# KumarRobotics/top_down_renderer

Hardware: AMD Instinct MI355X
Metric: particle-updates/sec (render+score+resample) (higher is better)
Workload: dtype f32

## Files before the change

include/tdr.h:

```cpp
#ifndef TDR_H_
#define TDR_H_

#include <stddef.h>
#include <stdint.h>

#ifdef __cplusplus
extern "C" {
#endif

#define TDR_OK 0
#define TDR_ERR_ARG (-1)
#define TDR_ERR_HIP (-2)
#define TDR_ERR_NOMEM (-3)

#define TDR_MAX_CLASSES 15
#define TDR_ST_FIELDS 7
enum { TDR_ST_INIT_X = 0, TDR_ST_INIT_Y = 1, TDR_ST_DX = 2, TDR_ST_DY = 3, TDR_ST_THETA = 4, TDR_ST_SCALE = 5,
       TDR_ST_HAVE_INIT = 6 };

typedef struct tdr_state {
  float init_x_px, init_y_px, dx_m, dy_m, theta, scale;
  uint8_t have_init;
  uint8_t pad_[3];
} tdr_state;
// ... 173 lines not shown
int tdr_k_local_map_polar(const tdr_map_desc* map, const float* tab, int nb, int nr, float cx, float cy, float scale,
                          float res, float* dists_out, uint8_t* mask_out, void* stream);
int tdr_k_local_map_cart(const tdr_map_desc* map, int rows, int cols, float cx, float cy, float rot, float res,
                         float* dists_out, uint8_t* mask_out, void* stream);

int tdr_k_active_diffs(const tdr_map_desc* map, const float* tab, int nb, int nr, float res, const float* centres,
                       const int32_t* shifts, int K, int ncand, double* sums_out, void* stream);
int tdr_active_candidates_host(const float* preds, int K, int nb, float* centres, float* dists, float* thetas,
                               int32_t* shifts, int* ntheta_out, int* ndist_out);

#define TDR_MEAN_COV_FLOATS 4800
int tdr_k_mean_cov(const float* st, int64_t cap, int64_t n, const float* about, float* out, void* stream);
int tdr_k_set_scale(float* st, int64_t cap, int64_t n, const float* scale_dev, void* stream);
int tdr_k_save_ml_state(const float* info, const float* st, int64_t cap, int64_t src_shard, int64_t n, float* out12,
                        void* stream);
int tdr_k_shift_init(float* st, int64_t cap, int64_t n, float dx, float dy, void* stream);

int tdr_config_compact(int on);
int tdr_config_shift_uniform(int mode);
float tdr_config_shift_uniform_span(float cells);
int tdr_config_ray_split(int k);
int tdr_config_cart_skip(int on);
int tdr_config_init_mfma(int on);
int tdr_config_uw_waves(int on);
int64_t tdr_shift_uniform_launches(void);

int tdr_profile_enable(int on);
int tdr_profile_score_ms(double* total_ms, int64_t* launches);
int tdr_profile_shares(double* dense_ms, double* scattered_ms, int64_t* scattered_particles);
int tdr_profile_variants(int64_t out[16]);

int64_t tdr_config_tuning(const char* name, int64_t value);
int tdr_su_tail_plan(int nchunks, int k, int q, int row, int* group, int* s0, int* s1);
int tdr_selftest_score(void);
int tdr_k_selftest_round(const float* x, int64_t n, float limit, int32_t* out, void* stream);
int tdr_libm_variant(void);
int tdr_libm_force_variant(int variant);
int tdr_sincosf_host(const float* x, int64_t n, int variant, float* sin_out, float* cos_out);
int tdr_k_selftest_sincos(const float* x, int64_t n, float* sin_out, float* cos_out, void* stream);
int tdr_logf_host(const float* x, int64_t n, float* out);
int tdr_k_selftest_logf(const float* x, int64_t n, float* out, void* stream);
int tdr_k_selftest_atan2(const float* y, const float* x, int64_t n, float* out, void* stream);

int tdr_k_states_aos_to_soa(const tdr_state* aos, int64_t n, float* st, int64_t cap, void* stream);
int tdr_k_states_soa_to_aos(const float* st, int64_t cap, int64_t n, tdr_state* aos, void* stream);
size_t tdr_locality_tmp_ints(int64_t n, int map_rows, int map_cols);
int tdr_k_locality_order(const float* st, int64_t cap, int64_t n, int map_rows, int map_cols, int32_t* perm_out,
                         int32_t* keys_tmp, void* stream);
size_t tdr_locality_pose_tmp_ints(int64_t n);
int tdr_k_locality_order_pose(const float* st, int64_t cap, int64_t n, int map_rows, int map_cols, float theta_radius,
                              int32_t* perm_out, int32_t* keys_tmp, void* stream);

typedef struct tdr_map tdr_map;
typedef struct tdr_renderer tdr_renderer;
typedef struct tdr_filter tdr_filter;

int tdr_map_create(tdr_map** out);
void tdr_map_destroy(tdr_map* m);
int tdr_map_set(tdr_map* m, const float* class_maps, const uint8_t* class_mask, int ncls, int rows, int cols,
                float resolution, int center_x, int center_y);
int tdr_map_set_labels(tdr_map* m, const uint8_t* label_img, int img_h, int img_w, const int32_t* flatten_lut,
                       int lut_size, int ncls, float resolution, int center_x, int center_y);
int tdr_map_update_labels_incremental(tdr_map* m, const uint8_t* label_img, int img_h, int img_w,
                                      const int32_t* flatten_lut, int lut_size, int ncls, float resolution, int center_x,
                                      int center_y, int64_t* changed_cells);
int tdr_map_patch_labels(tdr_map* m, const uint8_t* patch, int y0, int x0, int h, int w, int center_x, int center_y,
// ... 144 lines not shown
```

top_down_renderer_amd/_lib.py:

```python
import ctypes as C
import os

_PKG = os.path.dirname(os.path.abspath(__file__))
SO_PATH = os.environ.get("TDR_LIB_PATH") or os.path.join(_PKG, "libtdr_hip.so")

TDR_ST_FIELDS = 7
TDR_MAX_CLASSES = 15
TDR_SVG_NO_KEY = 0xFFFFFFFF


class FilterParamsC(C.Structure):
    _fields_ = [
        ("pos_cov", C.c_float), ("theta_cov", C.c_float), ("regularization", C.c_float),
        ("init_pos_px_x", C.c_float), ("init_pos_px_y", C.c_float), ("init_pos_px_cov", C.c_float),
        ("init_pos_m_x", C.c_float), ("init_pos_m_y", C.c_float),
        ("init_pos_deg_theta", C.c_float), ("init_pos_deg_cov", C.c_float),
        ("force_on_map", C.c_int32),
        ("fixed_scale", C.c_float), ("scale_log_min", C.c_float), ("scale_log_max", C.c_float),
        ("num_classes", C.c_int32),
        ("class_weights", C.c_float * 16),
    ]


class MapDescC(C.Structure):
# ... 79 lines not shown
    "tdr_raster_workspace_bytes": (_i64, [_i64]),
    "tdr_k_raster_polar": (_i, [_vp, _i, _i, _i64, _f, _f, _vp, _i, _i, _i, _vp, _vp, _vp, _vp]),
    "tdr_k_raster_cart": (_i, [_vp, _i, _i, _i64, _f, _vp, _i, _i, _i, _vp, _vp, _vp, _vp]),
    "tdr_raster_geo_workspace_bytes": (_i64, [_i64]),
    "tdr_k_raster_geo_polar": (_i, [_vp, _i, _i64, _i64, _f, _f, _i, _i, _vp, _vp, _vp]),
    "tdr_k_raster_geo_cart": (_i, [_vp, _i, _i64, _i64, _f, _i, _i, _vp, _vp]),
    "tdr_k_pack_scan": (_i, [_vp, _i, _i, _i, _vp, _vp]),
    "tdr_score_workspace_floats": (C.c_size_t, [_i, _i, _i, _i64, _i64]),
    "tdr_k_score_polar": (_i, [C.POINTER(MapDescC), _vp, _vp, _i, _i, _f, C.POINTER(FilterParamsC), _vp, _i64, _i64,
                               _i64, _vp, _f, _i, _vp, _vp, _vp]),
    "tdr_k_active_diffs": (_i, [C.POINTER(MapDescC), _vp, _i, _i, _f, _vp, _vp, _i, _i, _vp, _vp]),
    "tdr_active_candidates_host": (_i, [_vp, _i, _i, _vp, _vp, _vp, _vp, C.POINTER(_i), C.POINTER(_i)]),
    "tdr_logf_host": (_i, [_vp, _i64, _vp]),
    "tdr_k_selftest_logf": (_i, [_vp, _i64, _vp, _vp]),
    "tdr_rng_pipe_create": (_i, [_i64, C.POINTER(_vp)]),
    "tdr_rng_pipe_destroy": (None, [_vp]),
    "tdr_rng_pipe_on_device": (_i, [_vp]),
    "tdr_rng_pipe_from_host": (_i, [_vp, _vp, _vp]),
    "tdr_rng_pipe_to_host": (_i, [_vp, _vp, _vp]),
    "tdr_rng_pipe_normals": (_i, [_vp, _i64, _i64, _i64, _i, C.POINTER(_vp), _vp]),
    "tdr_rng_pipe_uniform": (_i, [_vp, C.POINTER(_vp), _vp]),
    "tdr_rng_dev_workspace_bytes": (C.c_size_t, [_i64]),
    "tdr_k_rng_propagate_normals": (_i, [_vp, _i64, _i64, _i64, _i, _vp, _vp, _vp]),
    "tdr_k_rng_uniform": (_i, [_vp, _vp, _vp]),
    "tdr_rng_get_state_host": (_i, [_vp, _vp]),
    "tdr_rng_set_state_host": (_i, [_vp, _vp]),
    "tdr_k_resample_dev": (_i, [_vp, _i64, _i64, _vp, _i64, _i64, _vp, _vp]),
    "tdr_score_ctx_create": (_i, [C.POINTER(_vp)]),
    "tdr_score_ctx_destroy": (None, [_vp]),
    "tdr_score_ctx_span": (C.c_float, [_vp]),
    "tdr_score_ctx_trial_calls": (_i64, [_vp]),
    "tdr_config_tuning": (_i64, [C.c_char_p, _i64]),
    "tdr_su_tail_plan": (_i, [_i, _i, _i, _i, C.POINTER(_i), C.POINTER(_i), C.POINTER(_i)]),
    "tdr_selftest_score": (_i, []),
    "tdr_profile_variants": (_i, [C.POINTER(_i64)]),
    "tdr_score_ctx_set_polar_factors": (_i, [_vp, _vp, _i, _i]),
    "tdr_polar_factors_host": (_i, [_i, _i, _f, _f, _vp]),
    "tdr_k_score_polar_ctx": (_i, [C.POINTER(MapDescC), _vp, _vp, _i, _i, _f, C.POINTER(FilterParamsC), _vp, _i64, _i64,
                                   _i64, _vp, _f, _i, _vp, _vp, _vp, _vp]),
    "tdr_score_geo_workspace_floats": (C.c_size_t, [_i, _i, _i, _i64, _i64]),
    "tdr_k_score_polar_geo": (_i, [C.POINTER(MapDescC), C.POINTER(MapDescC), _vp, _vp, _vp, _f, _f, _i, _i, _f,
                                   C.POINTER(FilterParamsC), _vp, _i64, _i64, _i64, _vp, _f, _i, _vp, _vp, _vp]),
    "tdr_score_cart_workspace_floats": (C.c_size_t, [_i, _i, _i, _i64, _i64]),
    "tdr_k_score_cart": (_i, [C.POINTER(MapDescC), _vp, _i, _i, _f, C.POINTER(FilterParamsC), _vp, _i64, _i64, _i64,
                              _vp, _vp, _vp, _vp]),
    "tdr_score_cart_init_workspace_floats": (C.c_size_t, [_i, _i, _i, _i64, _i64]),
    "tdr_k_score_cart_init": (_i, [C.POINTER(MapDescC), _vp, _i, _i, _f, C.POINTER(FilterParamsC), _vp, _i64, _i64, _i64,
                                   _vp, _vp]),
    "tdr_k_propagate": (_i, [_vp, _i64, _i64, _vp, _f, _f, _f, _i, _f, _f, _vp, _u64, _u64, _i64, _vp]),
    "tdr_rng_create": (_vp, [_u32]),
    "tdr_rng_destroy": (None, [_vp]),
    "tdr_rng_uniform_host": (_f, [_vp]),
    "tdr_propagate_normals_host": (_i, [_vp, _i64, _i, _vp]),
    "tdr_k_update_weights": (_i, [_vp, _vp, _i64, _vp, _vp, _vp]),
    "tdr_prefix_workspace_bytes": (_i64, [_i64]),
    "tdr_k_prefix": (_i, [_vp, _i64, _vp, _vp, _vp]),
    "tdr_k_prefix_mode": (_i, [_vp, _i64, _i, _vp, _vp, _vp, _vp]),
    "tdr_k_resample": (_i, [_vp, _i64, _i64, _f, _i64, _i64, _vp, _vp]),
    "tdr_k_gather_states": (_i, [_vp, _i64, _i64, _vp, _i64, _vp, _i64, _vp]),
    "tdr_init_particles_host": (_i, [_vp, _vp, _i, _i, _i, _f, C.POINTER(FilterParamsC), _i, _vp, C.POINTER(C.c_int64)]),
    "tdr_init_particles_count": (_i64, [C.POINTER(FilterParamsC), _i]),
    "tdr_init_workspace_bytes": (C.c_size_t, []),
    "tdr_k_init_particles": (_i, [_vp, C.POINTER(MapDescC), C.POINTER(FilterParamsC), _i, _i64, _i64, _vp, _i64,
                                  C.POINTER(C.c_int64), _vp, _vp]),
    "tdr_rng_pipe_init_particles": (_i, [_vp, C.POINTER(MapDescC), C.POINTER(FilterParamsC), _i, _i64, _i64, _vp, _i64,
                                         C.POINTER(C.c_int64), _vp, _vp]),
# ... 123 lines not shown
```

top_down_renderer_amd/csrc/tdr_score.hip:

```cpp

#include "tdr_common.h"
#include "tdr_batch.h"
#include "tdr_sincosf.h"

struct ScoreArgs {
  const float* rec;
  int rows, cols;
  float resolution;
  const float* tab;
  const float* utab = nullptr;
  const float* scan_pk;
  int nb, nr;
  float res;
  const float* st;
  int64_t cap, n;
  const int32_t* order;
  const int32_t* count = nullptr;
  const int32_t* slot_base = nullptr;
  int use_theta_override = 0;
  float theta_override = 0.f;
  int only_uninit = 0;
  int group, nchunks;
  int64_t npad;
  float* part;
// ... 591 lines not shown
      }
    cost = cost / (float)norm;
  }
  a.raw_w[p] = (float)(1. / (double)(cost + a.fp.regularization));
}

static int finalize_tlog(int nchunks, int64_t nslots) {
  int tl = 0;
  while (tl < 4 && (nchunks >> (tl + 1)) >= 4 && (nslots << (tl + 1)) <= 131072) tl++;
  return tl;
}
static void launch_finalize(FinalizeArgs& f, int64_t nslots, hipStream_t s) {
  f.tlog = finalize_tlog(f.nchunks, nslots);
  hipLaunchKernelGGL(score_finalize_kernel, dim3((unsigned)cdiv(nslots << f.tlog, 256)), dim3(256), 0, s, f);
}

#define TDR_CART_WAVE_MUL 2
static int64_t g_score_waves = 131072;
static int g_score_group = 0;
static int g_su_group = 0;
static int64_t score_wave_target() { return g_score_waves; }
extern "C" int tdr_config_init_ahead(int);
extern "C" int tdr_config_batch_init_search(int);
extern "C" int tdr_config_prefix_head(int);
extern "C" int tdr_config_ray_block_major(int);
extern "C" int tdr_config_ray_patch(int);
extern "C" int tdr_config_ray_borrow(int);
extern "C" int tdr_config_cart_seg_rows(int);
extern "C" int tdr_config_mt_stretches(int);
extern "C" int tdr_config_su_wave_span(int);
extern "C" int tdr_config_su_lds_pad(int);
extern "C" int tdr_config_su_tail_groups(int);
extern "C" int tdr_config_su_tail_parts(int);
extern "C" int tdr_config_init_device(int);
extern "C" int64_t tdr_config_init_window_words(int64_t);
extern "C" int64_t tdr_config_cart_init_chunk(int64_t);
extern "C" int64_t tdr_config_tuning(const char* name, int64_t value) {
  if (!name) return -1;
  const std::string n(name);
  if (n == "score_waves") { if (value > 0) g_score_waves = value; return g_score_waves; }
  if (n == "score_group") { if (value >= 0) g_score_group = (int)value; return g_score_group; }
  if (n == "su_group") { if (value >= 0) g_su_group = (int)value; return g_su_group; }
  if (n == "batch_init_search") return tdr_config_batch_init_search((int)std::max<int64_t>(value, -1));
  if (n == "init_ahead") return tdr_config_init_ahead((int)std::min<int64_t>(std::max<int64_t>(value, -1), 3));
  if (n == "prefix_head") return tdr_config_prefix_head((int)std::max<int64_t>(value, -1));
  if (n == "ray_borrow") return tdr_config_ray_borrow((int)std::max<int64_t>(value, -1));
  if (n == "ray_patch") return tdr_config_ray_patch((int)std::max<int64_t>(value, -1));
  if (n == "ray_block_major") return tdr_config_ray_block_major((int)std::max<int64_t>(value, -1));
  if (n == "cart_seg_rows") return tdr_config_cart_seg_rows((int)std::max<int64_t>(value, -1));
  if (n == "mt_stretches") return tdr_config_mt_stretches((int)std::max<int64_t>(value, -1));
  if (n == "su_lds_pad") return tdr_config_su_lds_pad((int)std::max<int64_t>(value, -1));
  if (n == "su_tail_groups") return tdr_config_su_tail_groups((int)std::min<int64_t>(std::max<int64_t>(value, -1), 1 << 20));
  if (n == "su_tail_parts") return tdr_config_su_tail_parts((int)std::min<int64_t>(std::max<int64_t>(value, -1), 8));
  if (n == "su_wave_span") return tdr_config_su_wave_span((int)std::max<int64_t>(value, -1));
  if (n == "init_device") return tdr_config_init_device((int)std::max<int64_t>(value, -1));
  if (n == "init_window_words") return tdr_config_init_window_words(value > 0 ? value : -1);
  if (n == "cart_init_chunk") return tdr_config_cart_init_chunk(value > 0 ? value : -1);
  return -1;
}
static void choose_chunks(int64_t n, int nr, int& rpc, int& nchunks, int target_mul = 1) {
  int64_t nbatches = cdiv(std::max<int64_t>(n, 1), 64);
  int64_t want = std::max<int64_t>(1, cdiv(score_wave_target() * target_mul, nbatches));
  nchunks = (int)std::min<int64_t>(nr, want);
  rpc = (int)cdiv(nr, nchunks);
  nchunks = (int)cdiv(nr, rpc);
}

__global__ void utab_kernel(const float* __restrict__ tab, int64_t n2, float scale, float res,
                            float* __restrict__ utab) {
  const int64_t k = (int64_t)blockIdx.x * blockDim.x + threadIdx.x;
  if (k < n2) utab[k] = (tab[k] * scale) * res;
}

static int score_group_rings(int nb, int nr, int rf, int64_t n_total) {
  const int forced = g_score_group;
  const int64_t ring_bytes = std::max<int64_t>((int64_t)nb * rf * 4, 1);
  int g = (int)std::min<int64_t>(8, (32 * 1024) / ring_bytes);
  const int64_t chunks_wanted = cdiv(2048, cdiv(std::max<int64_t>(n_total, 1), 256));
  g = (int)std::min<int64_t>(g, std::max<int64_t>(1, nr / std::max<int64_t>(chunks_wanted, 1)));
  if (forced > 0) g = forced;
  g = std::max(1, std::min<int>(g, (int)((60 * 1024) / ring_bytes)));
  if (g >= TDR_SCORE_U) g -= g % TDR_SCORE_U;
  return std::max(g, 1);
}
extern "C" int tdr_cmap_words(int ncls);
struct ScoreWs {
// ... 679 lines not shown
```

top_down_renderer_amd/csrc/tdr_score_su.h:

```cpp
#ifndef TDR_SCORE_SU_H_
#define TDR_SCORE_SU_H_
#include "tdr_common.h"

static inline int64_t su_npad(int64_t n, int nb) { return cdiv(n + 63 * std::min<int64_t>(nb, n), 64) * 64; }
bool tdr_su_shape_ok(int nb, int nr, int group, int64_t n_total);
struct SuWs {
  int64_t tab_su, desc, bbox, keys_in, keys_out, vals_in, vals_out, ints, slots, sort_tmp, ray_tab, ray_desc, ray_multi, ray_rad, total;
  int64_t slots2, wave_tmp;
};
#define TDR_SU_TAIL_INTS 10
#define TDR_RAY_MAX_SPLIT 8
SuWs tdr_su_ws(int nb, int nr, int group, int64_t n);

#define TDR_SU_NSECT 8
__host__ __device__ static inline int su_tail_plan(int nchunks, int k, int q, int row, int* group, int* s0, int* s1) {
  const int lq = q >= 8 ? 3 : (q >= 4 ? 2 : (q >= 2 ? 1 : 0));
  const int kk = k < 0 ? 0 : (k > nchunks ? nchunks : k);
  const int head = nchunks - kk, rows = head + (kk << lq);
  if (row < 0 || row >= rows) return rows;
  if (row < head) {
    *group = row; *s0 = 0; *s1 = TDR_SU_NSECT;
  } else {
    const int t = row - head, part = t & ((1 << lq) - 1);
    *group = head + (t >> lq);
    *s0 = part << (3 - lq);
    *s1 = (part + 1) << (3 - lq);
  }
  return rows;
}
void tdr_su_tail(int nchunks, int64_t n, int* k, int* q);

struct SuLaunch {
  const tdr_map_desc* map;
  const float* tab;
  bool uniform_scale;
  const float* scan_pk;
  int nb, nr, rf;
  float res;
  const float* st;
  int64_t cap, n;
  const int32_t* perm;
// ... 37 lines not shown
```

top_down_renderer_amd/csrc/tdr_score_su.hip:

```cpp
#include <rocprim/device/device_radix_sort.hpp>

#include <atomic>

#include "tdr_score_dev.h"
#include "tdr_score_su.h"
#include "tdr_score_su_asm.h"

#define SU_CODE_FULL 0xFFu
#define SU_CODE_FULL_ALL 0xFEu
#define SU_CODE_PAD 0xFDu
#define SU_NSECT TDR_SU_NSECT
#define SU_BOX_WORDS 4096

struct SuArgs {
  const uint32_t* crec;
  const uint32_t* kmask;
  int kcolw;
  unsigned kmask_off;
  const uint32_t* dict_int;
  int dict_n, ctiles_r;
  int pkcol;
  const int32_t* inexact;
  int rows, cols;
  float resolution;
// ... 67 lines not shown
  desc[4 * t + 2] = ckc;
  desc[4 * t + 3] = sh | (((jj & 3) == 0 && anyfull) ? 0x80000000u : 0u);
}

__global__ __launch_bounds__(256) void su_bbox_kernel(const float* __restrict__ tab_su, int nb, int nr, int group,
                                                      float* __restrict__ bbox) {
  const int chunk = blockIdx.x, sect = blockIdx.y;
  const int i0 = (int)((int64_t)sect * nb / SU_NSECT), i1 = (int)((int64_t)(sect + 1) * nb / SU_NSECT);
  const int gn = min(nr - chunk * group, group);
  float lo0 = 3.402823466e+38f, hi0 = -3.402823466e+38f, lo1 = lo0, hi1 = hi0;
  const int cnt = (i1 - i0) * gn;
  for (int t = threadIdx.x; t < cnt; t += 256) {
    const int i = i0 + t / gn, jj = t % gn;
    const float* e = tab_su + (((int64_t)chunk * nb + i) * group + jj) * 2;
    lo0 = fminf(lo0, e[0]); hi0 = fmaxf(hi0, e[0]);
    lo1 = fminf(lo1, e[1]); hi1 = fmaxf(hi1, e[1]);
  }
  __shared__ float red[4][256];
  red[0][threadIdx.x] = lo0; red[1][threadIdx.x] = hi0; red[2][threadIdx.x] = lo1; red[3][threadIdx.x] = hi1;
  __syncthreads();
  for (int d = 128; d > 0; d >>= 1) {
    if ((int)threadIdx.x < d) {
      red[0][threadIdx.x] = fminf(red[0][threadIdx.x], red[0][threadIdx.x + d]);
      red[1][threadIdx.x] = fmaxf(red[1][threadIdx.x], red[1][threadIdx.x + d]);
      red[2][threadIdx.x] = fminf(red[2][threadIdx.x], red[2][threadIdx.x + d]);
      red[3][threadIdx.x] = fmaxf(red[3][threadIdx.x], red[3][threadIdx.x + d]);
    }
    __syncthreads();
  }
  if (threadIdx.x < 4) bbox[((int64_t)chunk * SU_NSECT + sect) * 4 + threadIdx.x] = red[threadIdx.x][0];
}

__global__ __launch_bounds__(256) void su_key_kernel(const float* __restrict__ st, int64_t cap, int64_t n,
                                                     const int32_t* __restrict__ perm, int nb, float span,
                                                     uint32_t* __restrict__ keys, int32_t* __restrict__ vals,
                                                     int* __restrict__ cnt) {
  extern __shared__ int hist[];
  for (int k = threadIdx.x; k <= nb; k += 256) hist[k] = 0;
  __syncthreads();
  const int64_t t = (int64_t)blockIdx.x * blockDim.x + threadIdx.x;
  if (t < n) {
    const int32_t p = perm ? perm[t] : (int32_t)t;
    uint32_t key = (uint32_t)rot_shift_dev(st[TDR_ST_THETA * cap + p], nb);
    if (span > 0.f) {
      auto centre = [&](int64_t q, float& x, float& y) {
        const float sc = st[TDR_ST_SCALE * cap + q];
        x = st[TDR_ST_DX * cap + q] * sc + st[TDR_ST_INIT_X * cap + q];
        y = st[TDR_ST_DY * cap + q] * sc + st[TDR_ST_INIT_Y * cap + q];
      };
      const int64_t ta = t >= 32 ? t - 32 : 0, tb = t + 32 < n ? t + 32 : n - 1;
      float x0, y0, x1, y1;
      centre(perm ? perm[ta] : ta, x0, y0);
      centre(perm ? perm[tb] : tb, x1, y1);
      if (!(fabsf(x1 - x0) <= span && fabsf(y1 - y0) <= span)) key = (uint32_t)nb;
    }
    keys[t] = key;
    vals[t] = p;
    atomicAdd(&hist[key], 1);
  }
  __syncthreads();
  for (int k = threadIdx.x; k <= nb; k += 256)
    if (hist[k]) atomicAdd(&cnt[k], hist[k]);
}

__global__ __launch_bounds__(256) void su_offsets_kernel(const int* __restrict__ cnt, int nkeys, int* __restrict__ start,
                                                         int* __restrict__ slot_start, int* __restrict__ counts) {
  __shared__ int sa[256], sb[256];
  int carry_a = 0, carry_b = 0;
  for (int base = 0; base < nkeys; base += 256) {
    const int k = base + threadIdx.x;
    const int c = k < nkeys ? cnt[k] : 0;
    const int cp = k < nkeys - 1 ? (c + 63) & ~63 : c;
    sa[threadIdx.x] = c;
    sb[threadIdx.x] = cp;
    __syncthreads();
    for (int d = 1; d < 256; d <<= 1) {
      const int va = threadIdx.x >= d ? sa[threadIdx.x - d] : 0;
      const int vb = threadIdx.x >= d ? sb[threadIdx.x - d] : 0;
      __syncthreads();
      sa[threadIdx.x] += va;
      sb[threadIdx.x] += vb;
      __syncthreads();
    }
    if (k < nkeys) {
      start[k] = carry_a + sa[threadIdx.x] - c;
      slot_start[k] = carry_b + sb[threadIdx.x] - cp;
    }
    carry_a += sa[255];
    carry_b += sb[255];
    __syncthreads();
  }
  if (threadIdx.x == 0) {
    const int sparse = cnt[nkeys - 1];
    counts[0] = carry_b - sparse;
    counts[1] = sparse;
    counts[2] = carry_b;
  }
}

__global__ __launch_bounds__(256) void su_scatter_kernel(const uint32_t* __restrict__ keys, const int32_t* __restrict__ vals,
                                                         int64_t n, const int* __restrict__ start,
                                                         const int* __restrict__ slot_start, int32_t* __restrict__ slots) {
  const int64_t t = (int64_t)blockIdx.x * blockDim.x + threadIdx.x;
  if (t >= n) return;
  const uint32_t k = keys[t];
  slots[slot_start[k] + ((int)t - start[k])] = vals[t];
}

__global__ __launch_bounds__(256) void su_wave_far_kernel(const float* __restrict__ st, int64_t cap, const int32_t* __restrict__ slots,
                                                          const int32_t* __restrict__ counts, float wave_span,
                                                          int32_t* __restrict__ keep, int32_t* __restrict__ moved) {
  const int lane = threadIdx.x & 63;
  const int64_t w = (int64_t)blockIdx.x * 4 + (threadIdx.x >> 6), base = w * 64;
  if (base >= (int64_t)counts[0]) return;
  const int32_t p = slots[base + lane];
  float x0 = 3.0e38f, x1 = -3.0e38f, y0 = 3.0e38f, y1 = -3.0e38f;
  if (p >= 0) {
    const float sc = st[TDR_ST_SCALE * cap + p];
    const float x = st[TDR_ST_DX * cap + p] * sc + st[TDR_ST_INIT_X * cap + p];
    const float y = st[TDR_ST_DY * cap + p] * sc + st[TDR_ST_INIT_Y * cap + p];
    x0 = x1 = x;
    y0 = y1 = y;
  }
#pragma unroll
  for (int d = 32; d > 0; d >>= 1) {
    x0 = fminf(x0, __shfl_xor(x0, d)); x1 = fmaxf(x1, __shfl_xor(x1, d));
    y0 = fminf(y0, __shfl_xor(y0, d)); y1 = fmaxf(y1, __shfl_xor(y1, d));
  }
  const int nvalid = __popcll(__ballot(p >= 0));
  const bool far = (x1 - x0 > wave_span) || (y1 - y0 > wave_span);
  if (lane == 0) {
    keep[w] = far ? 0 : 1;
    moved[w] = far ? nvalid : 0;
  }
}
__global__ __launch_bounds__(256) void su_compact_offsets_kernel(int32_t* __restrict__ keep, int32_t* __restrict__ moved,
                                                                 int32_t* __restrict__ counts, int32_t* __restrict__ old_counts) {
  __shared__ int sa[256], sb[256];
  const int c0 = counts[0], c1 = counts[1], c2 = counts[2];
// ... 606 lines not shown
extern "C" int64_t tdr_shift_uniform_launches(void) { return g_su_launches.load(); }
bool tdr_su_shape_ok(int nb, int nr, int group, int64_t n_total) {
  if (g_su_mode == 0) return false;
  if (group % 4 != 0 || nb > 4095) return false;
  if (g_su_mode == 2) return true;
  if ((int64_t)nb * nr < 8192) return false;
  return n_total >= (int64_t)64 * nb;
}
static int g_su_tail_groups = 4, g_su_tail_parts = 4;
extern "C" int tdr_config_su_tail_groups(int k) {
  if (k >= 0) g_su_tail_groups = k;
  return g_su_tail_groups;
}
extern "C" int tdr_config_su_tail_parts(int q) {
  if (q >= 0) g_su_tail_parts = q >= 8 ? 8 : (q >= 4 ? 4 : (q >= 2 ? 2 : 1));
  return g_su_tail_parts;
}
void tdr_su_tail(int nchunks, int64_t n, int* k, int* q) {
  *k = std::min(g_su_tail_groups, nchunks);
  *q = g_su_tail_parts;
  if (g_su_mode != 2 && cdiv(std::max<int64_t>(n, 1), 256) * nchunks < 2 * 256 * 6) *k = 0;
  if (*k == 0 || *q == 1) { *k = 0; *q = 1; }
}
extern "C" int tdr_su_tail_plan(int nchunks, int k, int q, int row, int* group, int* s0, int* s1) {
  int g = 0, a = 0, b = 0;
  const int rows = su_tail_plan(nchunks, k, q, row, &g, &a, &b);
  if (row >= 0 && row < rows) {
    if (group) *group = g;
    if (s0) *s0 = a;
    if (s1) *s1 = b;
  }
  return rows;
}
static size_t su_sort_tmp_bytes(int64_t n) {
  size_t bytes = 0;
  uint32_t* k = nullptr;
  int32_t* v = nullptr;
  hipError_t e = rocprim::radix_sort_pairs(nullptr, bytes, k, k, v, v, (size_t)std::max<int64_t>(n, 1), 0u, 12u,
                                           (hipStream_t)0, false);
  if (e != hipSuccess || bytes == 0) bytes = (size_t)(n + 4096) * 16;
  return bytes;
}
SuWs tdr_su_ws(int nb, int nr, int group, int64_t n) {
  SuWs w;
  const int64_t nchunks = cdiv(nr, group), nbins = nchunks * nb * group;
  int64_t o = 0;
  auto take = [&](int64_t words) { const int64_t at = o; o += (words + 63) / 64 * 64; return at; };
  w.tab_su = take(2 * nbins);
  w.desc = take(4 * nbins);
  w.bbox = take(nchunks * SU_NSECT * 4);
  w.keys_in = take(n);
  w.keys_out = take(n);
  w.vals_in = take(n);
  w.vals_out = take(n);
  w.ints = take(3 * ((int64_t)nb + 1) + TDR_SU_TAIL_INTS);
  w.slots = take(su_npad(n, nb));
  w.slots2 = take(su_npad(n, nb));
  w.wave_tmp = take(2 * (su_npad(n, nb) / 64 + 1));
  w.sort_tmp = take((int64_t)((su_sort_tmp_bytes(n) + 3) / 4));
  const int64_t T = tdr_ray_padded_samples(nb, nr);
  w.ray_tab = take(2 * T);
  w.ray_desc = take((T + 1) / 2);
  w.ray_multi = take((int64_t)nb * nr);
  w.ray_rad = take(T / nb);
  w.total = o;
  return w;
}

int tdr_su_order(const SuLaunch& L, const SuWs& W, hipStream_t s, const int32_t** slots_out, const int32_t** counts_out) {
  int32_t* base = L.ws;
  uint32_t* keys_in = reinterpret_cast<uint32_t*>(base + W.keys_in);
  uint32_t* keys_out = reinterpret_cast<uint32_t*>(base + W.keys_out);
  int32_t* vals_in = base + W.vals_in;
  int32_t* vals_out = base + W.vals_out;
  int* cnt = base + W.ints;
  const int nkeys = L.nb + 1;
  int* start = cnt + nkeys;
  int* slot_start = start + nkeys;
  int* counts = slot_start + nkeys;
  int32_t* slots = base + W.slots;
  const int64_t n = L.n;
  HIP_TRY(hipMemsetAsync(cnt, 0, sizeof(int) * (size_t)(3 * nkeys + TDR_SU_TAIL_INTS), s));
  HIP_TRY(hipMemsetAsync(slots, 0xFF, sizeof(int32_t) * (size_t)L.npad, s));
  hipLaunchKernelGGL(su_key_kernel, dim3((unsigned)cdiv(n, 256)), dim3(256), sizeof(int) * (size_t)nkeys, s, L.st, L.cap, n,
                     L.perm, L.nb, L.span, keys_in, vals_in, cnt);
  LAUNCH_CHECK("su_key");
  hipLaunchKernelGGL(su_offsets_kernel, dim3(1), dim3(256), 0, s, (const int*)cnt, nkeys, start, slot_start, counts);
  LAUNCH_CHECK("su_offsets");
  unsigned bits = 1;
  while ((1u << bits) < (unsigned)nkeys) bits++;
  size_t tmp_bytes = su_sort_tmp_bytes(n);
  HIP_TRY(rocprim::radix_sort_pairs(base + W.sort_tmp, tmp_bytes, keys_in, keys_out, vals_in, vals_out, (size_t)n, 0u, bits,
                                    s, false));
  hipLaunchKernelGGL(su_scatter_kernel, dim3((unsigned)cdiv(n, 256)), dim3(256), 0, s, (const uint32_t*)keys_out,
                     (const int32_t*)vals_out, n, (const int*)start, (const int*)slot_start, slots);
  LAUNCH_CHECK("su_scatter");
  if (L.wave_span > 0.f && L.nb > 1) {
    int32_t* slots2 = base + W.slots2;
    int32_t* keep = base + W.wave_tmp;
    int32_t* moved = keep + (L.npad / 64 + 1);
    int32_t* old_counts = counts + 7;
    const int64_t nwaves = L.npad / 64;
    hipLaunchKernelGGL(su_wave_far_kernel, dim3((unsigned)cdiv(nwaves, 4)), dim3(256), 0, s, L.st, L.cap, (const int32_t*)slots,
                       (const int32_t*)counts, L.wave_span, keep, moved);
    hipLaunchKernelGGL(su_compact_offsets_kernel, dim3(1), dim3(256), 0, s, keep, moved, counts, old_counts);
    hipLaunchKernelGGL(su_compact_scatter_kernel, dim3((unsigned)cdiv(L.npad, 256)), dim3(256), 0, s, (const int32_t*)slots,
                       (const int32_t*)keep, (const int32_t*)moved, (const int32_t*)counts, (const int32_t*)old_counts, slots2);
    hipLaunchKernelGGL(su_copy_slots_kernel, dim3((unsigned)cdiv(L.npad, 256)), dim3(256), 0, s, (const int32_t*)slots2,
                       (const int32_t*)counts, slots);
    LAUNCH_CHECK("su_reroute");
  }
  *slots_out = slots;
  *counts_out = counts;
  return TDR_OK;
}
int tdr_su_prepare(const SuLaunch& L, const SuWs& W, hipStream_t s, const int32_t** slots_out, const int32_t** counts_out) {
  if (int rc = tdr_su_order(L, W, s, slots_out, counts_out)) return rc;
  int32_t* base = L.ws;
  float* tab_su = reinterpret_cast<float*>(base + W.tab_su);
  uint32_t* desc = reinterpret_cast<uint32_t*>(base + W.desc);
  const int64_t ndesc = (int64_t)L.nchunks * L.nb * L.group;
  const int lc = L.map->cwords == 1 ? 3 : (L.map->cwords == 2 ? 2 : 1);
  const int ckconst = ((L.map->rows >> lc) + 2) * 128 + 128;
  const unsigned plane_bytes = (unsigned)(tdr_cmap_plane_words(L.map->ncls, L.map->rows, L.map->cols) * 4);
  const unsigned pbase = (unsigned)(tdr_cmap_plane_offset_words(L.map->ncls, L.map->rows, L.map->cols) * 4) +
                         (unsigned)(plane_trows(L.map->rows) * 128) + 128u;
  hipLaunchKernelGGL(su_prep_kernel, dim3((unsigned)cdiv(ndesc, 256)), dim3(256), 0, s, L.tab, L.scan_pk, L.nb, L.nr, L.rf,
                     L.map->ncls, ckconst, pbase, plane_bytes, L.group, L.nchunks, L.map->dict, L.map->dict_n, tab_su, desc);
  LAUNCH_CHECK("su_prep");
  hipLaunchKernelGGL(su_bbox_kernel, dim3((unsigned)L.nchunks, SU_NSECT), dim3(256), 0, s, (const float*)tab_su, L.nb, L.nr,
                     L.group, reinterpret_cast<float*>(base + W.bbox));
  LAUNCH_CHECK("su_bbox");
  return TDR_OK;
}

int tdr_su_score(const SuLaunch& L, const SuWs& W, hipStream_t s) {
  const tdr_map_desc* map = L.map;
  int32_t* base = L.ws;
  int* nslots = base + W.ints + 3 * (L.nb + 1);
  SuArgs u;
  const int lc = map->cwords == 1 ? 3 : (map->cwords == 2 ? 2 : 1);
  u.crec = map->crec; u.dict_int = reinterpret_cast<const uint32_t*>(map->dict) + TDR_CMAP_MAX_DICT;
  u.dict_n = map->dict_n; u.ctiles_r = (map->rows >> lc) + 2;
  u.pkcol = plane_trows(map->rows) * 128 - 16;
  u.inexact = nslots + 4;
  u.rows = map->rows; u.cols = map->cols; u.resolution = map->resolution;
// ... 33 lines not shown
```

top_down_renderer_amd/kernels.py:

```python
import ctypes as C

import numpy as np
import torch

from . import _lib
from ._lib import FilterParamsC, MapDescC, check


def _ptr(t):
    return C.c_void_p(t.data_ptr()) if t is not None else C.c_void_p(0)


class ScoreCtx:

    def __init__(self, lib, handle):
        self.lib, self.handle = lib, handle

    def span(self):
        return float(self.lib.tdr_score_ctx_span(self.handle))

    def trial_calls(self):
        return int(self.lib.tdr_score_ctx_trial_calls(self.handle))

    def __del__(self):
# ... 531 lines not shown
        covs = np.zeros((max_k, 9), np.float32)
        check(self.lib.tdr_gmm_select_host(x.ctypes.data_as(C.c_void_p), len(x), int(num_particles), C.byref(k), max_k,
                                           means.ctypes.data_as(C.c_void_p), covs.ctypes.data_as(C.c_void_p)))
        return k.value, means[: k.value].copy(), covs[: k.value].reshape(-1, 3, 3).copy()

    def set_scale(self, st, n, scale_dev):
        check(self.lib.tdr_k_set_scale(_ptr(st), st.shape[1], n, _ptr(scale_dev), self.stream()))

    def shift_init(self, st, n, dx, dy):
        check(self.lib.tdr_k_shift_init(_ptr(st), st.shape[1], n, C.c_float(dx), C.c_float(dy), self.stream()))

    def locality_order(self, st, n, rows, cols, perm):
        need = int(self.lib.tdr_locality_tmp_ints(n, rows, cols))
        tmp = self.empty((need,), torch.int32)
        check(self.lib.tdr_k_locality_order(_ptr(st), st.shape[1], n, rows, cols, _ptr(perm), _ptr(tmp),
                                            self.stream()))

    def locality_order_pose(self, st, n, rows, cols, perm, theta_radius):
        need = int(self.lib.tdr_locality_pose_tmp_ints(n))
        tmp = self.empty((need + 2,), torch.int32)
        check(self.lib.tdr_k_locality_order_pose(_ptr(st), st.shape[1], n, rows, cols, C.c_float(theta_radius),
                                                 _ptr(perm), _ptr(tmp), self.stream()))

    def states_to_device(self, states_aos, st, n):
        raw = self.to_device(np.ascontiguousarray(states_aos).view(np.uint8).reshape(-1))
        check(self.lib.tdr_k_states_aos_to_soa(_ptr(raw), n, _ptr(st), st.shape[1], self.stream()))
        self.synchronize()

    def states_to_host(self, st, n, dtype):
        raw = self.empty((n * 28,), torch.uint8)
        check(self.lib.tdr_k_states_soa_to_aos(_ptr(st), st.shape[1], n, _ptr(raw), self.stream()))
        return raw.cpu().numpy().view(dtype).reshape(-1).copy()

    def tuning(self, name, value=-1):
        return int(self.lib.tdr_config_tuning(name.encode(), value))

    def rng_create(self, seed):
        return C.c_void_p(self.lib.tdr_rng_create(C.c_uint32(seed & 0xFFFFFFFF)))

    device_rng = True

    def rng_state_to_device(self, rng):
        words = np.zeros(640, np.uint32)
        check(self.lib.tdr_rng_get_state_host(rng, words.ctypes.data_as(C.c_void_p)))
        return self.to_device(words.view(np.int32))

    def rng_state_to_host(self, rng, state_dev):
        words = np.ascontiguousarray(state_dev.cpu().numpy()).view(np.uint32)
        check(self.lib.tdr_rng_set_state_host(rng, words.ctypes.data_as(C.c_void_p)))

    def rng_propagate_normals_dev(self, state_dev, n, lo, hi, scale_freeze, z4_out, n_max):
        need = int(self.lib.tdr_rng_dev_workspace_bytes(max(n, n_max)))
        if getattr(self, "_rws", None) is None or self._rws.numel() < need:
            self._rws = self.empty((need,), torch.uint8)
        check(self.lib.tdr_k_rng_propagate_normals(_ptr(state_dev), n, lo, hi, int(scale_freeze), _ptr(z4_out),
                                                   _ptr(self._rws), self.stream()))

    def rng_uniform_dev(self, state_dev, out_dev):
        check(self.lib.tdr_k_rng_uniform(_ptr(state_dev), _ptr(out_dev), self.stream()))

    def resample_dev(self, runmax, n, n_new, shift_dev, i_begin, i_end, idx):
        check(self.lib.tdr_k_resample_dev(_ptr(runmax), n, n_new, _ptr(shift_dev), i_begin, i_end, _ptr(idx), self.stream()))

    def rng_pipe_create(self, n_max):
        h = C.c_void_p(0)
        check(self.lib.tdr_rng_pipe_create(n_max, C.byref(h)))
# ... 28 lines not shown
```

Before: 23.08 million.

## Replace radix sort with segmented bucket histogram and ballot rank-scatter for particle ordering

Particle ordering by rotation bucket now uses a per-segment histogram table, a column prefix scan, and a wave-level ballot-based stable rank scatter, replacing the rocprim radix sort. Padding slots are filled to -1 in the offsets kernel, and the tail counters are cleared there too, so the two memsets go away. The aim is to cut the multi-pass radix sort and its launch overhead in the score preparation step. It costs an extra workspace table and adds a new debug entry point. A bucket-count-dependent fallback to the old path is kept.

```diff
diff --git a/include/tdr.h b/include/tdr.h
--- a/include/tdr.h
+++ b/include/tdr.h
@@ -229,6 +229,10 @@
 
 int64_t tdr_config_tuning(const char* name, int64_t value);
 int tdr_su_tail_plan(int nchunks, int k, int q, int row, int* group, int* s0, int* s1);
+size_t tdr_k_su_order_workspace_ints(int64_t n, int nb);
+int64_t tdr_k_su_order_slots(int64_t n, int nb);
+int tdr_k_su_order(const float* st, int64_t cap, int64_t n, const int32_t* perm, int nb, float span, int32_t* workspace,
+                   int32_t* slots_out, int32_t* keys_out, int32_t* counts_out, int* bucket_out, void* stream);
 int tdr_selftest_score(void);
 int tdr_k_selftest_round(const float* x, int64_t n, float limit, int32_t* out, void* stream);
 int tdr_libm_variant(void);
diff --git a/top_down_renderer_amd/_lib.py b/top_down_renderer_amd/_lib.py
--- a/top_down_renderer_amd/_lib.py
+++ b/top_down_renderer_amd/_lib.py
@@ -135,6 +135,9 @@
     "tdr_score_ctx_trial_calls": (_i64, [_vp]),
     "tdr_config_tuning": (_i64, [C.c_char_p, _i64]),
     "tdr_su_tail_plan": (_i, [_i, _i, _i, _i, C.POINTER(_i), C.POINTER(_i), C.POINTER(_i)]),
+    "tdr_k_su_order_workspace_ints": (C.c_size_t, [_i64, _i]),
+    "tdr_k_su_order_slots": (_i64, [_i64, _i]),
+    "tdr_k_su_order": (_i, [_vp, _i64, _i64, _vp, _i, _f, _vp, _vp, _vp, _vp, C.POINTER(_i), _vp]),
     "tdr_selftest_score": (_i, []),
     "tdr_profile_variants": (_i, [C.POINTER(_i64)]),
     "tdr_score_ctx_set_polar_factors": (_i, [_vp, _vp, _i, _i]),
diff --git a/top_down_renderer_amd/csrc/tdr_score.hip b/top_down_renderer_amd/csrc/tdr_score.hip
--- a/top_down_renderer_amd/csrc/tdr_score.hip
+++ b/top_down_renderer_amd/csrc/tdr_score.hip
@@ -647,6 +647,7 @@
 extern "C" int tdr_config_su_lds_pad(int);
 extern "C" int tdr_config_su_tail_groups(int);
 extern "C" int tdr_config_su_tail_parts(int);
+extern "C" int tdr_config_su_order_bucket(int);
 extern "C" int tdr_config_init_device(int);
 extern "C" int64_t tdr_config_init_window_words(int64_t);
 extern "C" int64_t tdr_config_cart_init_chunk(int64_t);
@@ -667,6 +668,7 @@
   if (n == "su_lds_pad") return tdr_config_su_lds_pad((int)std::max<int64_t>(value, -1));
   if (n == "su_tail_groups") return tdr_config_su_tail_groups((int)std::min<int64_t>(std::max<int64_t>(value, -1), 1 << 20));
   if (n == "su_tail_parts") return tdr_config_su_tail_parts((int)std::min<int64_t>(std::max<int64_t>(value, -1), 8));
+  if (n == "su_order_bucket") return tdr_config_su_order_bucket((int)std::max<int64_t>(value, -1));
   if (n == "su_wave_span") return tdr_config_su_wave_span((int)std::max<int64_t>(value, -1));
   if (n == "init_device") return tdr_config_init_device((int)std::max<int64_t>(value, -1));
   if (n == "init_window_words") return tdr_config_init_window_words(value > 0 ? value : -1);
diff --git a/top_down_renderer_amd/csrc/tdr_score_su.h b/top_down_renderer_amd/csrc/tdr_score_su.h
--- a/top_down_renderer_amd/csrc/tdr_score_su.h
+++ b/top_down_renderer_amd/csrc/tdr_score_su.h
@@ -7,6 +7,7 @@
 struct SuWs {
   int64_t tab_su, desc, bbox, keys_in, keys_out, vals_in, vals_out, ints, slots, sort_tmp, ray_tab, ray_desc, ray_multi, ray_rad, total;
   int64_t slots2, wave_tmp;
+  int64_t seg_hist;
 };
 #define TDR_SU_TAIL_INTS 10
 #define TDR_RAY_MAX_SPLIT 8
diff --git a/top_down_renderer_amd/csrc/tdr_score_su.hip b/top_down_renderer_amd/csrc/tdr_score_su.hip
--- a/top_down_renderer_amd/csrc/tdr_score_su.hip
+++ b/top_down_renderer_amd/csrc/tdr_score_su.hip
@@ -123,14 +123,15 @@
 }
 
 __global__ __launch_bounds__(256) void su_key_kernel(const float* __restrict__ st, int64_t cap, int64_t n,
-                                                     const int32_t* __restrict__ perm, int nb, float span,
+                                                     const int32_t* __restrict__ perm, int nb, float span, int per_block,
                                                      uint32_t* __restrict__ keys, int32_t* __restrict__ vals,
-                                                     int* __restrict__ cnt) {
+                                                     int* __restrict__ cnt, int* __restrict__ seg_hist) {
   extern __shared__ int hist[];
   for (int k = threadIdx.x; k <= nb; k += 256) hist[k] = 0;
   __syncthreads();
-  const int64_t t = (int64_t)blockIdx.x * blockDim.x + threadIdx.x;
-  if (t < n) {
+  for (int it = 0; it < per_block; it += 256) {
+    const int64_t t = (int64_t)blockIdx.x * per_block + it + threadIdx.x;
+    if (t >= n) break;
     const int32_t p = perm ? perm[t] : (int32_t)t;
     uint32_t key = (uint32_t)rot_shift_dev(st[TDR_ST_THETA * cap + p], nb);
     if (span > 0.f) {
@@ -150,12 +151,61 @@
     atomicAdd(&hist[key], 1);
   }
   __syncthreads();
-  for (int k = threadIdx.x; k <= nb; k += 256)
-    if (hist[k]) atomicAdd(&cnt[k], hist[k]);
+  if (seg_hist) {
+    int* row = seg_hist + (int64_t)blockIdx.x * (nb + 1);
+    for (int k = threadIdx.x; k <= nb; k += 256) row[k] = hist[k];
+  } else {
+    for (int k = threadIdx.x; k <= nb; k += 256)
+      if (hist[k]) atomicAdd(&cnt[k], hist[k]);
+  }
+}
+
+#define SU_SEG 512
+#define SU_COLSCAN_WAVES 16
+__global__ __launch_bounds__(64 * SU_COLSCAN_WAVES) void su_colscan_kernel(int* __restrict__ seg_hist, int segs, int nkeys,
+                                                                           int* __restrict__ cnt) {
+  __shared__ int wsum[SU_COLSCAN_WAVES][64];
+  const int lane = threadIdx.x & 63, w = threadIdx.x >> 6;
+  const int k = blockIdx.x * 64 + lane;
+  const bool live = k < nkeys;
+  const int per = (segs + SU_COLSCAN_WAVES - 1) / SU_COLSCAN_WAVES;
+  const int s0 = min(w * per, segs), s1 = min(s0 + per, segs);
+  int* col = seg_hist + (live ? k : 0);
+  int sum = 0;
+  if (live)
+    for (int sgm = s0; sgm < s1; sgm += 8) {
+      int v[8];
+#pragma unroll
+      for (int u = 0; u < 8; u++) v[u] = sgm + u < s1 ? col[(int64_t)(sgm + u) * nkeys] : 0;
+#pragma unroll
+      for (int u = 0; u < 8; u++) sum += v[u];
+    }
+  wsum[w][lane] = sum;
+  __syncthreads();
+  int run = 0, tot = 0;
+#pragma unroll
+  for (int j = 0; j < SU_COLSCAN_WAVES; j++) {
+    const int v = wsum[j][lane];
+    run += j < w ? v : 0;
+    tot += v;
+  }
+  if (!live) return;
+  if (w == 0) cnt[k] = tot;
+  for (int sgm = s0; sgm < s1; sgm += 8) {
+    int v[8];
+#pragma unroll
+    for (int u = 0; u < 8; u++) v[u] = sgm + u < s1 ? col[(int64_t)(sgm + u) * nkeys] : 0;
+#pragma unroll
+    for (int u = 0; u < 8; u++) {
+      if (sgm + u < s1) col[(int64_t)(sgm + u) * nkeys] = run;
+      run += v[u];
+    }
+  }
 }
 
 __global__ __launch_bounds__(256) void su_offsets_kernel(const int* __restrict__ cnt, int nkeys, int* __restrict__ start,
-                                                         int* __restrict__ slot_start, int* __restrict__ counts) {
+                                                         int* __restrict__ slot_start, int* __restrict__ counts,
+                                                         int32_t* __restrict__ pad_slots) {
   __shared__ int sa[256], sb[256];
   int carry_a = 0, carry_b = 0;
   for (int base = 0; base < nkeys; base += 256) {
@@ -176,6 +226,8 @@
     if (k < nkeys) {
       start[k] = carry_a + sa[threadIdx.x] - c;
       slot_start[k] = carry_b + sb[threadIdx.x] - cp;
+      if (pad_slots)
+        for (int j = c; j < cp; j++) pad_slots[carry_b + sb[threadIdx.x] - cp + j] = -1;
     }
     carry_a += sa[255];
     carry_b += sb[255];
@@ -187,6 +239,7 @@
     counts[1] = sparse;
     counts[2] = carry_b;
   }
+  if (pad_slots && threadIdx.x >= 3 && threadIdx.x < TDR_SU_TAIL_INTS) counts[threadIdx.x] = 0;
 }
 
 __global__ __launch_bounds__(256) void su_scatter_kernel(const uint32_t* __restrict__ keys, const int32_t* __restrict__ vals,
@@ -196,6 +249,56 @@
   if (t >= n) return;
   const uint32_t k = keys[t];
   slots[slot_start[k] + ((int)t - start[k])] = vals[t];
+}
+
+__global__ __launch_bounds__(64) void su_rank_scatter_kernel(const uint32_t* __restrict__ keys, const int32_t* __restrict__ vals,
+                                                             int64_t n, const int* __restrict__ seg_pre,
+                                                             const int* __restrict__ slot_start, int nkeys, int bits,
+                                                             int32_t* __restrict__ slots) {
+  extern __shared__ int ctr[];
+  const int lane = threadIdx.x;
+  const int64_t t0 = (int64_t)blockIdx.x * SU_SEG;
+  uint32_t key[SU_SEG / 64];
+  int32_t val[SU_SEG / 64];
+#pragma unroll
+  for (int it = 0; it < SU_SEG / 64; it++) {
+    const int64_t t = t0 + it * 64 + lane;
+    key[it] = t < n ? keys[t] : 0u;
+    val[it] = t < n ? vals[t] : 0;
+  }
+  const int* row = seg_pre + (int64_t)blockIdx.x * nkeys;
+  for (int k0 = lane; k0 < nkeys; k0 += 256) {
+    int a[4], b[4];
+#pragma unroll
+    for (int u = 0; u < 4; u++) {
+      const int k = k0 + 64 * u;
+      a[u] = k < nkeys ? slot_start[k] : 0;
+      b[u] = k < nkeys ? row[k] : 0;
+    }
+#pragma unroll
+    for (int u = 0; u < 4; u++)
+      if (k0 + 64 * u < nkeys) ctr[k0 + 64 * u] = a[u] + b[u];
+  }
+  __syncthreads();
+#pragma unroll
+  for (int it = 0; it < SU_SEG / 64; it++) {
+    const bool live = t0 + it * 64 + lane < n;
+    uint64_t same = __ballot(live);
+    for (int b = 0; b < bits; b++) {
+      const bool one = (key[it] >> b) & 1u;
+      const uint64_t ones = __ballot(one);
+      same &= one ? ones : ~ones;
+    }
+    const int below = __popcll(same & (((uint64_t)1 << lane) - 1)), all = __popcll(same);
+    int at = 0;
+    if (live) {
+      at = ctr[key[it]];
+      slots[at + below] = val[it];
+    }
+    __syncthreads();
+    if (live && below == all - 1) ctr[key[it]] = at + all;
+    __syncthreads();
+  }
 }
 
 __global__ __launch_bounds__(256) void su_wave_far_kernel(const float* __restrict__ st, int64_t cap, const int32_t* __restrict__ slots,
@@ -868,6 +971,20 @@
   }
   return rows;
 }
+static int g_su_order_bucket = 1;
+extern "C" int tdr_config_su_order_bucket(int v) {
+  if (v >= 0) g_su_order_bucket = v ? 1 : 0;
+  return g_su_order_bucket;
+}
+static int64_t su_seg_table_words(int nb, int64_t n) {
+  const int64_t words = cdiv(std::max<int64_t>(n, 1), SU_SEG) * ((int64_t)nb + 1);
+  return words <= 4 * std::max<int64_t>(n, 1) + 65536 ? words : 0;
+}
+static int64_t su_seg_table_reserve(int nb, int64_t n) {
+  const int64_t m = std::max<int64_t>(n, 1);
+  return std::min<int64_t>(cdiv(m, SU_SEG) * ((int64_t)nb + 1), 4 * m + 65536);
+}
+static bool su_order_is_bucket(int nb, int64_t n) { return g_su_order_bucket && su_seg_table_words(nb, n) > 0; }
 static size_t su_sort_tmp_bytes(int64_t n) {
   size_t bytes = 0;
   uint32_t* k = nullptr;
@@ -899,6 +1016,7 @@
   w.ray_desc = take((T + 1) / 2);
   w.ray_multi = take((int64_t)nb * nr);
   w.ray_rad = take(T / nb);
+  w.seg_hist = take(su_seg_table_reserve(nb, n));
   w.total = o;
   return w;
 }
@@ -916,21 +1034,41 @@
   int* counts = slot_start + nkeys;
   int32_t* slots = base + W.slots;
   const int64_t n = L.n;
-  HIP_TRY(hipMemsetAsync(cnt, 0, sizeof(int) * (size_t)(3 * nkeys + TDR_SU_TAIL_INTS), s));
-  HIP_TRY(hipMemsetAsync(slots, 0xFF, sizeof(int32_t) * (size_t)L.npad, s));
-  hipLaunchKernelGGL(su_key_kernel, dim3((unsigned)cdiv(n, 256)), dim3(256), sizeof(int) * (size_t)nkeys, s, L.st, L.cap, n,
-                     L.perm, L.nb, L.span, keys_in, vals_in, cnt);
-  LAUNCH_CHECK("su_key");
-  hipLaunchKernelGGL(su_offsets_kernel, dim3(1), dim3(256), 0, s, (const int*)cnt, nkeys, start, slot_start, counts);
-  LAUNCH_CHECK("su_offsets");
-  unsigned bits = 1;
-  while ((1u << bits) < (unsigned)nkeys) bits++;
-  size_t tmp_bytes = su_sort_tmp_bytes(n);
-  HIP_TRY(rocprim::radix_sort_pairs(base + W.sort_tmp, tmp_bytes, keys_in, keys_out, vals_in, vals_out, (size_t)n, 0u, bits,
-                                    s, false));
-  hipLaunchKernelGGL(su_scatter_kernel, dim3((unsigned)cdiv(n, 256)), dim3(256), 0, s, (const uint32_t*)keys_out,
-                     (const int32_t*)vals_out, n, (const int*)start, (const int*)slot_start, slots);
-  LAUNCH_CHECK("su_scatter");
+  if (su_order_is_bucket(L.nb, n)) {
+    int* seg_hist = base + W.seg_hist;
+    const int64_t segs = cdiv(n, SU_SEG);
+    hipLaunchKernelGGL(su_key_kernel, dim3((unsigned)segs), dim3(256), sizeof(int) * (size_t)nkeys, s, L.st, L.cap, n, L.perm,
+                       L.nb, L.span, SU_SEG, keys_in, vals_in, (int*)nullptr, seg_hist);
+    LAUNCH_CHECK("su_key");
+    hipLaunchKernelGGL(su_colscan_kernel, dim3((unsigned)cdiv(nkeys, 64)), dim3(64 * SU_COLSCAN_WAVES), 0, s, seg_hist,
+                       (int)segs, nkeys, cnt);
+    LAUNCH_CHECK("su_colscan");
+    hipLaunchKernelGGL(su_offsets_kernel, dim3(1), dim3(256), 0, s, (const int*)cnt, nkeys, start, slot_start, counts, slots);
+    LAUNCH_CHECK("su_offsets");
+    unsigned bits = 1;
+    while ((1u << bits) < (unsigned)nkeys) bits++;
+    hipLaunchKernelGGL(su_rank_scatter_kernel, dim3((unsigned)segs), dim3(64), sizeof(int) * (size_t)nkeys, s,
+                       (const uint32_t*)keys_in, (const int32_t*)vals_in, n, (const int*)seg_hist, (const int*)slot_start, nkeys,
+                       (int)bits, slots);
+    LAUNCH_CHECK("su_rank_scatter");
+  } else {
+    HIP_TRY(hipMemsetAsync(cnt, 0, sizeof(int) * (size_t)(3 * nkeys + TDR_SU_TAIL_INTS), s));
+    HIP_TRY(hipMemsetAsync(slots, 0xFF, sizeof(int32_t) * (size_t)L.npad, s));
+    hipLaunchKernelGGL(su_key_kernel, dim3((unsigned)cdiv(n, 256)), dim3(256), sizeof(int) * (size_t)nkeys, s, L.st, L.cap, n,
+                       L.perm, L.nb, L.span, 256, keys_in, vals_in, cnt, (int*)nullptr);
+    LAUNCH_CHECK("su_key");
+    hipLaunchKernelGGL(su_offsets_kernel, dim3(1), dim3(256), 0, s, (const int*)cnt, nkeys, start, slot_start, counts,
+                       (int32_t*)nullptr);
+    LAUNCH_CHECK("su_offsets");
+    unsigned bits = 1;
+    while ((1u << bits) < (unsigned)nkeys) bits++;
+    size_t tmp_bytes = su_sort_tmp_bytes(n);
+    HIP_TRY(rocprim::radix_sort_pairs(base + W.sort_tmp, tmp_bytes, keys_in, keys_out, vals_in, vals_out, (size_t)n, 0u, bits,
+                                      s, false));
+    hipLaunchKernelGGL(su_scatter_kernel, dim3((unsigned)cdiv(n, 256)), dim3(256), 0, s, (const uint32_t*)keys_out,
+                       (const int32_t*)vals_out, n, (const int*)start, (const int*)slot_start, slots);
+    LAUNCH_CHECK("su_scatter");
+  }
   if (L.wave_span > 0.f && L.nb > 1) {
     int32_t* slots2 = base + W.slots2;
     int32_t* keep = base + W.wave_tmp;
@@ -948,6 +1086,30 @@
   }
   *slots_out = slots;
   *counts_out = counts;
+  return TDR_OK;
+}
+extern "C" size_t tdr_k_su_order_workspace_ints(int64_t n, int nb) {
+  if (n < 1 || nb < 1 || nb > 4095) return 0;
+  return (size_t)tdr_su_ws(nb, 4, 4, n).total;
+}
+extern "C" int64_t tdr_k_su_order_slots(int64_t n, int nb) { return n < 1 || nb < 1 ? 0 : su_npad(n, nb); }
+extern "C" int tdr_k_su_order(const float* st, int64_t cap, int64_t n, const int32_t* perm, int nb, float span,
+                              int32_t* workspace, int32_t* slots_out, int32_t* keys_out, int32_t* counts_out, int* bucket_out,
+                              void* stream) {
+  if (!st || !workspace || !slots_out || !keys_out || !counts_out) return fail(TDR_ERR_ARG, "su_order: null pointer");
+  if (n < 1 || cap < n || nb < 1 || nb > 4095) return fail(TDR_ERR_ARG, "su_order: bad shape");
+  hipStream_t s = (hipStream_t)stream;
+  const SuWs W = tdr_su_ws(nb, 4, 4, n);
+  SuLaunch L{};
+  L.st = st; L.cap = cap; L.n = n; L.perm = perm; L.nb = nb; L.span = span; L.ws = workspace;
+  L.npad = su_npad(n, nb);
+  const int32_t* slots = nullptr;
+  const int32_t* counts = nullptr;
+  if (bucket_out) *bucket_out = su_order_is_bucket(nb, n) ? 1 : 0;
+  if (int rc = tdr_su_order(L, W, s, &slots, &counts)) return rc;
+  HIP_TRY(hipMemcpyAsync(slots_out, slots, sizeof(int32_t) * (size_t)L.npad, hipMemcpyDeviceToDevice, s));
+  HIP_TRY(hipMemcpyAsync(keys_out, workspace + W.keys_in, sizeof(int32_t) * (size_t)n, hipMemcpyDeviceToDevice, s));
+  HIP_TRY(hipMemcpyAsync(counts_out, counts, sizeof(int32_t) * 3, hipMemcpyDeviceToDevice, s));
   return TDR_OK;
 }
 int tdr_su_prepare(const SuLaunch& L, const SuWs& W, hipStream_t s, const int32_t** slots_out, const int32_t** counts_out) {
diff --git a/top_down_renderer_amd/kernels.py b/top_down_renderer_amd/kernels.py
--- a/top_down_renderer_amd/kernels.py
+++ b/top_down_renderer_amd/kernels.py
@@ -587,6 +587,21 @@
         check(self.lib.tdr_k_states_soa_to_aos(_ptr(st), st.shape[1], n, _ptr(raw), self.stream()))
         return raw.cpu().numpy().view(dtype).reshape(-1).copy()
 
+    def su_order(self, st, n, nb, span, perm=None, workspace=None):
+        need = int(self.lib.tdr_k_su_order_workspace_ints(n, nb))
+        if workspace is None:
+            workspace = self.empty((need,), torch.int32)
+        if workspace.numel() < need:
+            raise ValueError(f"su_order: workspace of {workspace.numel()} words, {need} needed")
+        slots = self.empty((int(self.lib.tdr_k_su_order_slots(n, nb)),), torch.int32)
+        keys = self.empty((n,), torch.int32)
+        counts = self.empty((3,), torch.int32)
+        bucket = C.c_int(-1)
+        check(self.lib.tdr_k_su_order(_ptr(st), st.shape[1], n, _ptr(perm) if perm is not None else None, nb,
+                                      C.c_float(span), _ptr(workspace), _ptr(slots), _ptr(keys), _ptr(counts), C.byref(bucket),
+                                      self.stream()))
+        return slots, keys, counts, bool(bucket.value)
+
     def tuning(self, name, value=-1):
         return int(self.lib.tdr_config_tuning(name.encode(), value))
 
```

Measured after the change: 23.46 million (median of 6 runs). +1.6%, better.
